# MyersGroup/relate

Measured on AMD Instinct MI355X. Metric: haplotype-pair*SNP updates/sec (Paint), higher is better.
Workload: dtype f64; 1 GPU; synthetic block-coalescent panel, N=5000 haplotypes x L=500000 SNPs, 1 chunk per GPU, 267 windows (--memory 20), Paint = PaintSteppingStones for all targets; sum_mode=exact, sum_k_D_k=264261546

## Files before the change

### include/relate_amd.h

```cpp
#ifndef RELATE_AMD_H
#define RELATE_AMD_H

#include <stddef.h>
#include <stdint.h>

#ifdef __cplusplus
extern "C" {
#endif

enum {
  RL_OK = 0,
  RL_EINVAL = -1,
  RL_ENODEVICE = -2,
  RL_EHIP = -3,
  RL_EIO = -4,
  RL_EFORMAT = -5,
  RL_ESTATE = -6,
  RL_ENOMEM = -7,
  RL_ETIMEOUT = -8
};

enum { RL_SUM_EXACT = 0, RL_SUM_LANES = 1, RL_SUM_EXACT_SERIAL = 2, RL_SUM_LANES32 = 3 };

typedef struct rl_ctx rl_ctx;
typedef struct rl_window rl_window;

const char *rl_last_error(void);
const char *rl_version(void);
int rl_device_count(void);

rl_ctx *rl_create(int device);
void rl_keep_cache_until_exit(int on);
void rl_destroy(rl_ctx *ctx);

int rl_load_chunk(rl_ctx *ctx, const char *dir, int chunk_index);

int rl_set_chunk(rl_ctx *ctx, int N, int L, const uint8_t *seq,
                 const double *r, const double *rpos, const int *wb, int W);
int rl_set_chunk_bits(rl_ctx *ctx, int N, int L, const uint32_t *bits,
                      int row_words, const double *r, const double *rpos,
                      const int *wb, int W);

int rl_set_painting(rl_ctx *ctx, double theta, double rho);

int rl_set_target_range(rl_ctx *ctx, int k_begin, int k_end);
int rl_target_range(const rl_ctx *ctx, int *k_begin, int *k_end);

int rl_set_window_range(rl_ctx *ctx, int w_first, int w_last);
int rl_window_range(const rl_ctx *ctx, int *w_first, int *w_last);

int rl_chunk_dims(const rl_ctx *ctx, int *N, int *L, int *W);
long long rl_total_sites(rl_ctx *ctx);

int rl_prepare(rl_ctx *ctx);

int rl_paint(rl_ctx *ctx, int sum_mode, float *kernel_ms);
int rl_set_paint_split(rl_ctx *ctx, int split);
int rl_set_paint_fit(rl_ctx *ctx, int fit);
int rl_set_paint_segments(rl_ctx *ctx, int backward, int forward);
int rl_paint_segments(rl_ctx *ctx, int *backward, int *forward);
int rl_paint_launched_segments(const rl_ctx *ctx, int *backward, int *forward);
int rl_paint_segment_range(int lo, int hi, int seg, int s, int *first, int *last);
int rl_tile_fit(int N, int *S, int *waves, int *tail, int *live);
int rl_paint_times(const rl_ctx *ctx, float *fwd_ms, float *bwd_ms);
int rl_paint_account(const rl_ctx *ctx, long long *fwd_steps, long long *bwd_steps, long long *stone_bytes);
int rl_register_tile(const rl_ctx *ctx, int *S, int *waves);

#define RL_DEBUG_SUM_STASH 0x100
#define RL_DEBUG_SUM_REGSTASH 0x200
int rl_debug_wave_sum(const double *x, int n, int batch, int sum_mode, double *out);
int rl_debug_wave_sum_ex(const double *x, int n, int batch, int rows_per_group, int sum_mode,
                         const uint8_t *mismatch, double th, double nth, double *out,
                         unsigned long long *stats8);
int rl_debug_term_split(int S, int *ks, int *r);
int rl_debug_walk_table(const int *A4, int p0, int sh, int delta_lo, int delta_hi, int *packable, int *out_table,
                        int *out_reference);

int rl_debug_stats(rl_ctx *ctx, unsigned long long *out16);
int rl_debug_stats32(rl_ctx *ctx, unsigned long long *out32);
int rl_debug_timeline(rl_ctx *ctx, unsigned long long *out, long long cap, long long *groups);

int rl_get_stones(rl_ctx *ctx, int w, float *alpha, float *beta,
                  float *ls_alpha, float *ls_beta, int *bsnp_begin,
                  int *bsnp_end);

int rl_write_paint_files(rl_ctx *ctx, const char *paint_dir);
int rl_write_paint_file(rl_ctx *ctx, int w, const char *path);
int rl_paint_record(rl_ctx *ctx, int w, int k, unsigned char *out, size_t cap, size_t *len);

int rl_stage_paint(const char *out_dir, int chunk_index, int use_painting,
                   double theta, double rho, int sum_mode, int device);

rl_window *rl_window_open(rl_ctx *ctx, int w, const char *paint_file,
                          int first_snp, int sum_mode, float *kernel_ms);
rl_window *rl_window_open_bounded(rl_ctx *ctx, int w, const char *paint_file,
                                  int first_snp, int sum_mode,
                                  long long max_rows, float *kernel_ms);
int rl_window_repaints(const rl_window *win);
void rl_window_close(rl_window *win);
int rl_window_bounds(const rl_window *win, int *start, int *end);
int rl_window_rows(const rl_window *win, int n);
int rl_window_get_topology(rl_window *win, int n, float *top,
                           float *logscales);

int rl_window_advance(rl_window *win, int snp);
int rl_window_matrix(rl_window *win, int snp, float *d_host, float *kernel_ms);
int rl_window_matrix_rows_device(rl_window *win, int snp, void *d_rows, float *kernel_ms);
int rl_window_matrix_rows_device_ex(rl_window *win, int snp, void *d_rows, const char *carriers, float val,
                                    void *d_rowmin, float *kernel_ms);

int rl_quickbuild(int N, double theta, float *d, const float *d_prior,
                  int *parent, int *child_left, int *child_right);
typedef struct rl_builder rl_builder;
rl_builder *rl_builder_create(int N, double theta, int device);
int rl_builder_build(rl_builder *b, float *d, const float *d_prior,
                     int *parent, int *child_left, int *child_right);
int rl_builder_set_sample_ages(rl_builder *b, const double *ages, int n);
int rl_builder_last_on_gpu(const rl_builder *b);
void rl_builder_destroy(rl_builder *b);
int rl_debug_rng_mismatches(unsigned seed, int n);
int rl_debug_builder_throughput(int N, double theta, int device, int builders, int reps, int workers, const float *d,
                                const float *prior, double *seconds, int *mismatches, int *first_parents);
int rl_debug_stage_worker_goal(int cus, int open_sections, int bounded_windows, int workers_per_cu);
int rl_debug_stage_plan(int N, int nloc, int S, int waves, const double *rows_of, int num_windows, int first_section,
                        int last_section, int stones_per_window, int gpu_build, int room_known, double room,
                        int host_threads, int window_rows_set, long long window_rows, long long window_parts,
                        int section_threads_set, long long section_threads, long long repaint_lanes, int probe_section,
                        long long *ints_out, double *doubles_out);

typedef struct rl_treeseq rl_treeseq;
typedef int (*rl_matrix_fn)(void *user, int snp, float *d);
typedef int (*rl_advance_fn)(void *user, int snp);
rl_treeseq *rl_treeseq_create(int N, int L, const uint32_t *bits, int row_words,
                              const double *rpos, const int *bp_pos,
                              const int *state, double theta);
void rl_treeseq_destroy(rl_treeseq *ts);
int rl_treeseq_set_sample_ages(rl_treeseq *ts, const double *ages, int n);
int rl_treeseq_set_build_device(rl_treeseq *ts, int device);
typedef int (*rl_matrix_dev_fn)(void *user, int snp, void *d_dev);
int rl_treeseq_set_device_matrix(rl_treeseq *ts, rl_matrix_dev_fn matrix_dev);
typedef int (*rl_matrix_dev_ex_fn)(void *user, int snp, void *d_matrix, const char *carriers, float val,
                                   void *d_rowmin);
int rl_treeseq_set_device_matrix_ex(rl_treeseq *ts, rl_matrix_dev_ex_fn matrix_dev_ex);
int rl_treeseq_build(rl_treeseq *ts, int start, int end, rl_matrix_fn matrix,
                     rl_advance_fn advance, void *user, int flags, int fb);
int rl_treeseq_num_trees(const rl_treeseq *ts);
int rl_treeseq_get_tree(const rl_treeseq *ts, int t, int *pos, int *parent);
int rl_treeseq_write(const rl_treeseq *ts, const char *anc_path,
                     const char *mut_path);

int rl_stage_build_topology(const char *out_dir, int chunk_index,
                            int first_section, int last_section,
                            int use_painting, double theta, double rho,
                            int flags, int fb, int sum_mode, int device);

typedef struct rl_stage_opts {
  size_t size;
  int sum_mode;
  int device;
// ... 123 lines not shown
```

### relate_amd/api.py

```python
import ctypes as C
import os

import numpy as np

_HERE = os.path.dirname(os.path.abspath(__file__))
LIB_PATH = os.path.join(_HERE, "librelate_amd.so")

RL_SUM_EXACT = 0
RL_SUM_LANES = 1
RL_SUM_EXACT_SERIAL = 2
RL_SUM_LANES32 = 3
RL_DEBUG_SUM_STASH = 0x100
RL_DEBUG_SUM_REGSTASH = 0x200

_lib = None


class RelateError(RuntimeError):
    pass


def lib():
    global _lib
    if _lib is None:
# ... 40 lines not shown
                                        C.c_void_p, C.POINTER(C.c_longlong)]
        L.rl_pairwise_anc.restype = C.c_int
        L.rl_pairwise_anc.argtypes = [C.POINTER(C.c_char_p), C.c_int, C.c_int, C.c_int, C.c_void_p,
                                      C.POINTER(C.c_longlong), C.POINTER(C.c_int)]
        L.rl_coalrate_batch_trees.argtypes = [C.c_int]
        L.rl_coalrate_epochs.argtypes = [C.c_float, C.c_char_p, C.c_void_p, C.POINTER(C.c_int)]
        L.rl_coalrate_trees.argtypes = [C.c_void_p, C.c_void_p, C.c_void_p, C.c_int, C.c_int, C.c_void_p, C.c_int,
                                        C.c_int, C.c_void_p]
        L.rl_coalrate_anc.argtypes = [C.c_char_p, C.c_char_p, C.c_void_p, C.c_int, C.c_int, C.c_void_p,
                                      C.POINTER(C.c_int)]
        L.rl_coalrate_write_bin.argtypes = [C.c_char_p, C.c_void_p, C.c_int, C.c_void_p, C.c_int]
        L.rl_coalrate_read_bin.argtypes = [C.c_char_p, C.c_void_p, C.POINTER(C.c_int), C.c_void_p, C.POINTER(C.c_int)]
        L.rl_coalrate_finalize.argtypes = [C.c_void_p, C.c_int, C.c_int, C.c_void_p, C.c_int, C.c_void_p]
        L.rl_coalrate_finalize_files.argtypes = [C.c_char_p, C.c_char_p, C.c_char_p]
        L.rl_window_copying.argtypes = [C.c_void_p, C.c_void_p, C.c_void_p]
        L.rl_window_copying_host.argtypes = [C.c_void_p, C.c_void_p, C.c_void_p]
        L.rl_copying_matrix.argtypes = [C.c_void_p, C.c_int, C.c_int, C.c_int, C.c_void_p, C.POINTER(C.c_longlong)]
        L.rl_copying_weights_host.argtypes = [C.c_void_p, C.c_int, C.c_void_p, C.c_int, C.c_int, C.c_void_p]
        L.rl_copying_rows_host.argtypes = [C.c_void_p, C.c_void_p, C.c_int, C.c_int, C.c_void_p]
        L.rl_stage_copying_matrix.argtypes = [C.c_char_p, C.c_int, C.c_int, C.c_int, C.c_void_p, C.c_char_p]
        _lib = L
    return _lib


class PaintTimeout(RelateError):
    """RL_ETIMEOUT: a segmented paint() gave up waiting for a hand-off"""


RL_ETIMEOUT = -8


def _check(rc):
    if rc == RL_ETIMEOUT:
        raise PaintTimeout("librelate_amd error %d: %s" % (rc, lib().rl_last_error().decode()))
    if rc != 0:
        raise RelateError("librelate_amd error %d: %s" % (rc, lib().rl_last_error().decode()))


def _p(a):
    return None if a is None else a.ctypes.data_as(C.c_void_p)


def device_count():
    return lib().rl_device_count()


def debug_wave_sum(x, sum_mode, rows_per_group=1, mismatch=None, th=0.001, nth=0.999, stash=False, regstash=False):
    if stash:
        sum_mode |= RL_DEBUG_SUM_STASH
    if regstash:
        sum_mode |= RL_DEBUG_SUM_REGSTASH
    x = np.ascontiguousarray(x, dtype=np.float64)
    batch, n = x.shape
    if mismatch is not None:
        mismatch = np.ascontiguousarray(mismatch, dtype=np.uint8)
        assert mismatch.shape == x.shape
    out = np.empty(batch, np.float64)
    st = np.zeros(8, np.uint64)
    f = lib().rl_debug_wave_sum_ex
    f.argtypes = [C.c_void_p, C.c_int, C.c_int, C.c_int, C.c_int, C.c_void_p, C.c_double, C.c_double, C.c_void_p,
                  C.c_void_p]
    _check(f(_p(x), n, batch, rows_per_group, sum_mode, _p(mismatch), th, nth, _p(out), _p(st)))
    return out, {"sums": int(st[0]), "fallbacks": int(st[1]), "walked": int(st[2]), "reruns": int(st[3])}


def term_split(S):
    ks, r = C.c_int(), C.c_int()
    _check(lib().rl_debug_term_split(int(S), C.byref(ks), C.byref(r)))
    return ks.value, r.value


def walk_table(A4, p0, sh, delta_lo, delta_hi):
    A4 = np.ascontiguousarray(A4, dtype=np.int32)
    assert A4.shape == (4,)
    n = int(delta_hi) - int(delta_lo) + 1
    tab, ref = np.empty(max(n, 0), np.int32), np.empty(max(n, 0), np.int32)
    ok = C.c_int()
    f = lib().rl_debug_walk_table
    f.argtypes = [C.c_void_p, C.c_int, C.c_int, C.c_int, C.c_int, C.POINTER(C.c_int), C.c_void_p, C.c_void_p]
    _check(f(_p(A4), int(p0), int(sh), int(delta_lo), int(delta_hi), C.byref(ok), _p(tab), _p(ref)))
    return bool(ok.value), tab, ref


def paint_segment_range(lo, hi, seg, s):
    a, b = C.c_int(), C.c_int()
    _check(lib().rl_paint_segment_range(int(lo), int(hi), int(seg), int(s), C.byref(a), C.byref(b)))
    return a.value, b.value


def tile_fit(N):
    s, w, t, l = C.c_int(), C.c_int(), C.c_int(), C.c_int()
    _check(lib().rl_tile_fit(int(N), C.byref(s), C.byref(w), C.byref(t), C.byref(l)))
    return s.value, w.value, t.value, l.value


class Context:

    def __init__(self, device=0):
        self._h = lib().rl_create(device)
        if not self._h:
            raise RelateError(lib().rl_last_error().decode())
        self.N = self.L = self.W = 0

    def close(self):
        if self._h:
            lib().rl_destroy(self._h)
            self._h = None

    def __del__(self):
        self.close()

    def _dims(self):
        n, l, w = C.c_int(), C.c_int(), C.c_int()
        _check(lib().rl_chunk_dims(C.c_void_p(self._h), C.byref(n), C.byref(l), C.byref(w)))
        self.N, self.L, self.W = n.value, l.value, w.value

    def load_chunk(self, out_dir, chunk_index=0):
        _check(lib().rl_load_chunk(C.c_void_p(self._h), out_dir.encode(), chunk_index))
        self._dims()

    def set_chunk(self, seq, r, rpos, wb):
        seq = np.ascontiguousarray(seq, dtype=np.uint8)
        L, N = seq.shape
        r = np.ascontiguousarray(r, dtype=np.float64)
        rpos = np.ascontiguousarray(rpos, dtype=np.float64)
        wb = np.ascontiguousarray(wb, dtype=np.int32)
        assert len(r) == L and len(rpos) == L + 1
        _check(lib().rl_set_chunk(C.c_void_p(self._h), N, L, _p(seq), _p(r), _p(rpos), _p(wb), len(wb) - 1))
        self._dims()

    def set_chunk_bits(self, N, bits, r, rpos, wb):
        bits = np.ascontiguousarray(bits, dtype=np.uint32)
        L, rw = bits.shape
        r = np.ascontiguousarray(r, dtype=np.float64)
        rpos = np.ascontiguousarray(rpos, dtype=np.float64)
        wb = np.ascontiguousarray(wb, dtype=np.int32)
        _check(lib().rl_set_chunk_bits(C.c_void_p(self._h), N, L, _p(bits), rw, _p(r), _p(rpos), _p(wb),
                                       len(wb) - 1))
        self._dims()

    def set_painting(self, theta, rho):
        _check(lib().rl_set_painting(C.c_void_p(self._h), theta, rho))

    def set_target_range(self, k_begin, k_end):
        _check(lib().rl_set_target_range(C.c_void_p(self._h), int(k_begin), int(k_end)))

    def target_range(self):
        a, b = C.c_int(), C.c_int()
        _check(lib().rl_target_range(C.c_void_p(self._h), C.byref(a), C.byref(b)))
        return a.value, b.value

    def set_window_range(self, w_first, w_last):
        _check(lib().rl_set_window_range(C.c_void_p(self._h), int(w_first), int(w_last)))

    def window_range(self):
        a, b = C.c_int(), C.c_int()
        _check(lib().rl_window_range(C.c_void_p(self._h), C.byref(a), C.byref(b)))
        return a.value, b.value

    def paint_account(self):
        f, b, n = C.c_longlong(0), C.c_longlong(0), C.c_longlong(0)
        _check(lib().rl_paint_account(C.c_void_p(self._h), C.byref(f), C.byref(b), C.byref(n)))
        return f.value, b.value, n.value

    def total_sites(self):
        v = lib().rl_total_sites(C.c_void_p(self._h))
# ... 603 lines not shown
```

### relate_amd/csrc/debug_kernels.hip

```cpp
#define RL_STATS 1
#include "paint_device.h"
#include "exact_sum.h"
#include "launch.h"
#include "common.h"

#include <vector>

namespace rl {

constexpr int SUM_STATS = 8;

enum { TERM_REG = 0, TERM_MASK = 1, TERM_STASH = 2, TERM_REGSTASH = 3 };

template <int S, int MODE, int WAVES, int KIND>
__global__ void __launch_bounds__(64 * WAVES) sum_kernel(const double *__restrict__ x, int n, int rows_per_group,
                                                         const unsigned long long *__restrict__ masks, double th,
                                                         double nth, double *__restrict__ out,
                                                         unsigned long long *__restrict__ stats) {
  __shared__ WaveLinkStorage link;
  __shared__ unsigned long long lstats[SUM_STATS];
  constexpr bool STASHING = KIND == TERM_STASH || KIND == TERM_REGSTASH;
  constexpr int STASH = STASHING ? stash_bytes(S) : 16;
  constexpr int R = KIND == TERM_REGSTASH ? reg_stash_terms(S) : 0;
  __shared__ __attribute__((aligned(16))) char stash[WAVES][STASH];
// ... 106 lines not shown
  const Layout lay = make_layout(n, waves);
  const int S = choose_S(lay);
  if (!S) {
    set_error("rl_debug_wave_sum_ex: no register tile for n=%d", n);
    return RL_EINVAL;
  }
  std::vector<unsigned long long> masks;
  if (mismatch) {
    masks.assign((size_t)batch * waves * S, 0ull);
    for (size_t b = 0; b < (size_t)batch; b++)
      for (int vl = 0; vl < 64 * waves; vl++) {
        const int start = vl * lay.q + (vl < lay.rem ? vl : lay.rem), len = lay.q + (vl < lay.rem ? 1 : 0);
        unsigned long long *words = &masks[(b * waves + vl / 64) * S];
        for (int j = 0; j < len; j++)
          if (mismatch[b * n + start + j]) words[j] |= 1ull << (vl & 63);
      }
  }
  DevBuf dx, dout, dmask, dstats;
  int rc;
  if ((rc = dx.alloc(sizeof(double) * (size_t)n * batch))) return rc;
  if ((rc = dout.alloc(sizeof(double) * batch))) return rc;
  if ((rc = dstats.alloc(sizeof(unsigned long long) * SUM_STATS))) return rc;
  if (mismatch && (rc = dmask.alloc(sizeof(unsigned long long) * masks.size()))) return rc;
  RL_HIP(hipMemcpy(dx.p, x, sizeof(double) * (size_t)n * batch, hipMemcpyHostToDevice));
  RL_HIP(hipMemset(dstats.p, 0, sizeof(unsigned long long) * SUM_STATS));
  if (mismatch)
    RL_HIP(hipMemcpy(dmask.p, masks.data(), sizeof(unsigned long long) * masks.size(), hipMemcpyHostToDevice));
  const unsigned long long *dm = mismatch ? dmask.as<unsigned long long>() : nullptr;
  const int groups = batch / rows_per_group;
  hipError_t e;
  switch (kernel_mode(sum_mode)) {
#define RL_ARGS S, waves, dx.as<double>(), n, groups, rows_per_group, dm, th, nth, dout.as<double>(), \
                dstats.as<unsigned long long>(), kind
    case 0: e = launch_sum<0>(RL_ARGS); break;
    case 1: e = launch_sum<1>(RL_ARGS); break;
    default: e = launch_sum<2>(RL_ARGS); break;
#undef RL_ARGS
  }
  RL_HIP(e);
  RL_HIP(hipDeviceSynchronize());
  RL_HIP(hipMemcpy(out, dout.p, sizeof(double) * batch, hipMemcpyDeviceToHost));
  if (stats8) RL_HIP(hipMemcpy(stats8, dstats.p, sizeof(unsigned long long) * SUM_STATS, hipMemcpyDeviceToHost));
  return RL_OK;
}

extern "C" int rl_debug_wave_sum(const double *x, int n, int batch, int sum_mode, double *out) {
  return rl_debug_wave_sum_ex(x, n, batch, 1, sum_mode, nullptr, 0.0, 0.0, out, nullptr);
}

extern "C" int rl_debug_term_split(int S, int *ks, int *r) {
  using namespace rl;
  const hipError_t e = dispatch_tile(S, 1, [&](auto s, auto, auto) {
    *ks = stash_terms(s());
    *r = reg_stash_terms(s());
    return hipSuccess;
  });
  if (e != hipSuccess) {
    set_error("rl_debug_term_split: no register tile S=%d", S);
    return RL_EINVAL;
  }
  return RL_OK;
}

extern "C" int rl_debug_walk_table(const int *A4, int p0, int sh, int delta_lo, int delta_hi, int *packable,
                                   int *out_table, int *out_reference) {
  using namespace rl;
  if (!A4 || !packable || !out_table || !out_reference) {
    set_error("rl_debug_walk_table: null argument");
    return RL_EINVAL;
  }
  if (p0 < 0 || p0 > 3 || sh < 0 || sh > 1 || delta_hi < delta_lo) {
    set_error("rl_debug_walk_table: p0=%d outside 0..3, sh=%d outside 0..1 or delta_hi=%d < delta_lo=%d", p0, sh,
              delta_hi, delta_lo);
    return RL_EINVAL;
  }
  const WalkTable t = walk_table_pack(A4[0], A4[1], A4[2], A4[3], p0, sh);
  *packable = t.ok ? 1 : 0;
  for (long long d = delta_lo; d <= delta_hi; d++) {
    out_reference[d - delta_lo] = walk_hop_reference(A4[0], A4[1], A4[2], A4[3], p0, sh, (int)d);
    out_table[d - delta_lo] = t.ok ? walk_table_hop(t.lo, t.hi, 16 * p0, sh, (int)d) : 0;
  }
  return RL_OK;
}
```

### relate_amd/csrc/exact_sum.h

```cpp
#pragma once
#include "paint_device.h"

namespace rl {

template <int CTRL, int ROW_MASK = 0xf, int BANK_MASK = 0xf>
RL_DEV double dpp_f64(double v) {
  const long long b = __double_as_longlong(v);
  const int lo = __builtin_amdgcn_update_dpp(0, (int)b, CTRL, ROW_MASK, BANK_MASK, true);
  const int hi = __builtin_amdgcn_update_dpp(0, (int)(b >> 32), CTRL, ROW_MASK, BANK_MASK, true);
  return __longlong_as_double(((long long)hi << 32) | (unsigned int)lo);
}
template <int CTRL, int ROW_MASK = 0xf, int BANK_MASK = 0xf>
RL_DEV int dpp_i32(int v) {
  return __builtin_amdgcn_update_dpp(0, v, CTRL, ROW_MASK, BANK_MASK, true);
}
enum { DPP_ROW_SHR = 0x110, DPP_WAVE_SHR1 = 0x138, DPP_ROW_BCAST15 = 0x142, DPP_ROW_BCAST31 = 0x143 };

RL_DEV double wave_scan_f64(double v) {
  v += dpp_f64<DPP_ROW_SHR + 1>(v);
  v += dpp_f64<DPP_ROW_SHR + 2>(v);
  v += dpp_f64<DPP_ROW_SHR + 4>(v);
  v += dpp_f64<DPP_ROW_SHR + 8>(v);
  v += dpp_f64<DPP_ROW_BCAST15, 0xa>(v);
  v += dpp_f64<DPP_ROW_BCAST31, 0xc>(v);
  return v;
}
RL_DEV int hi32(double v) { return (int)(__double_as_longlong(v) >> 32); }
RL_DEV int expo_field(double v) { return (hi32(v) >> 20) & 0x7ff; }
RL_DEV double rd_lane_f64(double v, int lane) {
  const long long b = __double_as_longlong(v);
  const int lo = __builtin_amdgcn_readlane((int)b, lane);
  const int hi = __builtin_amdgcn_readlane((int)(b >> 32), lane);
  return __longlong_as_double(((long long)hi << 32) | (unsigned int)lo);
}
RL_DEV double pow2_field(int f) { return __longlong_as_double((long long)f << 52); }

template <int S, int LIVE = S>
struct RegTerm {
  static constexpr bool REG = true;
  const double (&a)[S];
  double th = 0.0, nth = 0.0;
  unsigned long long *stats = nullptr;
  RL_DEV double get(int i, double, double) const { return a[i]; }
  template <typename F>
  RL_DEV void for_each(double &, double &, F &&f) const {
#pragma unroll
    for (int i = 0; i < LIVE; i++) f(i, a[i]);
  }
};
template <int S, int LIVE = S>
struct MaskTerm {
  static constexpr bool REG = false;
  MaskRow row;
  const double (&b)[S];
  double th, nth;
  unsigned long long *stats = nullptr;
  template <typename F>
  RL_DEV void for_each(double &t, double &n, F &&f) const {
    for_each_chunk<S, 4>(row, [&](int j0, const u64x4 &m) {
      double x[4];
      if (j0 + 4 <= LIVE)
        weighted4(x, b[j0], b[j0 + 1], b[j0 + 2], b[j0 + 3], m, t, n);
      else
        weighted3(x, b[j0], b[j0 + 1], b[j0 + 2], m, t, n);
#pragma unroll
      for (int jj = 0; jj < 4; jj++)
        if (j0 + jj < LIVE) f(j0 + jj, x[jj]);
    });
  }
};

constexpr int STASH_MAX = 36;
constexpr int LDS_PER_CU = 160 * 1024;
constexpr int stash_terms(int S) {
  const int fit = (LDS_PER_CU / (4 * tile_waves_per_simd(S)) - 512) / (64 * (int)sizeof(double));
  const int ks = fit < S ? fit : S;
  return (ks < STASH_MAX ? ks : STASH_MAX) / 4 * 4;
}
constexpr int stash_bytes(int S) { return stash_terms(S) * 64 * (int)sizeof(double); }
constexpr int reg_stash_terms(int S) { return S == 80 ? 12 : S == 64 ? 28 : 0; }
template <int S, int R>
RL_DEV void hold_term(double (&xr)[R > 0 ? R : 1], int i, double x) {
  if constexpr (R > 0)
    if (i >= S - R) xr[i - (S - R)] = x;
}
constexpr int STASH_AHEAD = 2;
typedef double f64x2 __attribute__((ext_vector_type(2)));
typedef f64x2 __attribute__((may_alias)) StashPair;
typedef __attribute__((address_space(3))) StashPair *StashPtr;
RL_DEV StashPtr stash_of(void *wave_region) { return (StashPtr)wave_region + (threadIdx.x & 63); }
RL_DEV void stash_put4(StashPtr sp, int chunk, const double (&x)[4]) {
  StashPair lo, hi;
  lo.x = x[0]; lo.y = x[1]; hi.x = x[2]; hi.y = x[3];
  sp[128 * chunk] = lo;
  sp[128 * chunk + 64] = hi;
}
RL_DEV void stash_put3(StashPtr sp, int chunk, const double (&x)[4]) {
  StashPair lo;
  lo.x = x[0]; lo.y = x[1];
  sp[128 * chunk] = lo;
  *(__attribute__((address_space(3))) double __attribute__((may_alias)) *)&sp[128 * chunk + 64] = x[2];
}
template <int S, int LIVE = S, int R = reg_stash_terms(S)>
struct StashTerm {
  static constexpr bool REG = false;
  static constexpr int KS = stash_terms(S);
  static_assert(R % 4 == 0 && KS + R <= S, "the register-held chunks lie behind the stashed ones");
// ... 70 lines not shown
  lk.w = WAVES > 1 ? __builtin_amdgcn_readfirstlane((int)(threadIdx.x >> 6)) : 0;
  return lk;
}
template <int WAVES>
RL_DEV double lanes_total(double lane_sum, WaveLink<WAVES> &lk) {
  lk.phase++;
  const double t = wave_sum_butterfly(lane_sum);
  if constexpr (WAVES == 1) {
    return t;
  } else {
    const unsigned ph = lk.phase & 1u;
    if ((threadIdx.x & 63) == 0) lk.s->tot[ph][lk.w] = t;
    lk.barrier();
    return lk.s->tot[ph][0] + lk.s->tot[ph][1];
  }
}

template <int S, typename T>
RL_DEV double sum_exact_fallback(const T &term, double s = 0.0) {
  for (int l = 0; l < 64; l++) {
    double th = term.th, nth = term.nth;
    double tmp = s;
    term.for_each(th, nth, [&](int, double x) {
      tmp += x;
      if constexpr (!T::REG) asm volatile("" : "+v"(th), "+v"(nth), "+v"(tmp));
    });
    s = wave_bcast(tmp, l);
  }
  return s;
}
template <int S, int WAVES, typename T>
RL_DEV double sum_exact_fallback_linked(const T &term, const WaveLink<WAVES> &lk) {
  if constexpr (WAVES == 1) {
    return sum_exact_fallback<S>(term);
  } else {
    double r = 0.0;
    if (lk.w == 0) {
      r = sum_exact_fallback<S>(term);
      if ((threadIdx.x & 63) == 0) lk.s->result = r;
    }
    lk.barrier();
    if (lk.w == 1) {
      r = sum_exact_fallback<S>(term, lk.s->result);
    }
    lk.barrier();
    if (lk.w == 1 && (threadIdx.x & 63) == 0) lk.s->result = r;
    lk.barrier();
    r = lk.s->result;
    lk.barrier();
    return r;
  }
}

constexpr int WALK_G4 = 16384;
RL_HD inline int walk_hop_reference(int A0, int A1, int A2, int A3, int p0, int sh, int delta) {
  const int h = (p0 + delta) & 3;
  const int A = (h & 2) ? ((h & 1) ? A3 : A2) : ((h & 1) ? A1 : A0);
  const int B = h == 0 ? (-p0 - WALK_G4) : (h == 3 ? (3 - p0 + WALK_G4) : (h - p0));
  return A + ((delta - B) >> sh);
}
RL_HD inline int walk_run_offset(int A, int h, int p0, int sh) {
  const int B = h - p0 + (h == 0 ? -WALK_G4 : h == 3 ? WALK_G4 : 0);
  return A - (B >> sh);
}
struct WalkTable {
  int lo, hi;
  bool ok;
};
RL_HD inline WalkTable walk_table_pack_runs(int U0, int U1, int U2, int U3) {
  WalkTable t;
  t.ok = (short)U0 == U0 && (short)U1 == U1 && (short)U2 == U2 && (short)U3 == U3;
  t.lo = (int)(((unsigned)U0 & 0xffffu) | ((unsigned)U1 << 16));
  t.hi = (int)(((unsigned)U2 & 0xffffu) | ((unsigned)U3 << 16));
  return t;
}
RL_HD inline WalkTable walk_table_pack(int A0, int A1, int A2, int A3, int p0, int sh) {
  return walk_table_pack_runs(walk_run_offset(A0, 0, p0, sh), walk_run_offset(A1, 1, p0, sh),
                              walk_run_offset(A2, 2, p0, sh), walk_run_offset(A3, 3, p0, sh));
}
RL_HD inline int walk_table_hop(int lo, int hi, int p16, int sh, int delta) {
  const unsigned long long t = ((unsigned long long)(unsigned)hi << 32) | (unsigned)lo;
  return (delta >> sh) + (int)(short)(unsigned short)(t >> (((delta << 4) + p16) & 48));
}

#ifdef RL_STATS
#define RL_CLK() __builtin_readcyclecounter()
#define RL_STAT(i, v) do { if (term.stats && (threadIdx.x & 63) == 0) atomicAdd(&term.stats[i], (unsigned long long)(v)); } while (0)
#else
#define RL_CLK() 0ull
#define RL_STAT(i, v) do { } while (0)
#endif

template <int S, int WAVES, typename T>
RL_DEV double sum_exact_fast(const T &term, double L, WaveLink<WAVES> &lk) {
  constexpr bool REG_TERM = T::REG;
  constexpr int G4 = WALK_G4;

  const unsigned long long tk0 = RL_CLK();
  double Q = wave_scan_f64(L);
  double P = dpp_f64<DPP_WAVE_SHR1>(Q);
  if constexpr (WAVES > 1) {
    const int lane = threadIdx.x & 63;
    const unsigned ph = lk.phase & 1u;
    if (lane == 63) lk.s->tot[ph][lk.w] = Q;
    lk.barrier();
    if (lk.w == 1) {
      const double before = lk.s->tot[ph][0];
      Q = before + Q;
      P = dpp_f64<DPP_WAVE_SHR1>(Q);
      if (lane == 0) P = before;
    }
  }
  const long long pb = __double_as_longlong(P);
  const bool zero_entry = pb == 0 || ((threadIdx.x & 63) == 1 && lk.w == 0);

  const unsigned long long tk1 = RL_CLK();
  const long long base = pb & ~3ll;
  const int p0 = (int)(pb & 3);
  double c0 = __longlong_as_double(base - G4);
  double c1 = __longlong_as_double(base + 1);
  double c2 = __longlong_as_double(base + 2);
  double c3 = __longlong_as_double(base + 3 + G4);
  if (zero_entry) { c0 = P; c1 = P; c2 = P; c3 = P; }
  const double r0 = c0, r3 = c3;
  const int e_in = expo_field(r0);
  const bool entry_ok = zero_entry || (e_in == expo_field(r3) && e_in > 64);
  int exdiff = 0;
  double thB = term.th, nthB = term.nth;
  term.for_each(thB, nthB, [&](int, double x) {
    c0 += x;
    c1 += x;
    c2 += x;
    c3 += x;
    exdiff = __builtin_amdgcn_bitop3_b32(exdiff, hi32(c0), hi32(c3), 0xF6);
    if constexpr (REG_TERM)
      __builtin_amdgcn_sched_barrier(0);
    else
      asm volatile("" : "+v"(exdiff), "+v"(c1), "+v"(c2), "+v"(thB), "+v"(nthB));
  });
  const unsigned long long tk2 = RL_CLK();
  const int e_out = expo_field(c0);
  const int e_next = expo_field(Q);
  const unsigned q_lo = (unsigned)__double_as_longlong(Q);
  auto exit_offset = [&](double c) -> int { return (int)((unsigned)__double_as_longlong(c) - q_lo); };

  const bool same_seq = (exdiff >> 20) == 0;
  const int sh = e_out - e_in;
  bool invalid = !entry_ok || !same_seq;
  if (!zero_entry && e_out != e_next) invalid = true;
  if (zero_entry && expo_field(c0) != e_next) invalid = true;
  const bool jump = !zero_entry && !invalid && sh >= 2;
  const bool constant = jump && __double_as_longlong(c0) == __double_as_longlong(c3);
  const bool special = jump && !constant;

  int A0 = 0;
  if (constant) A0 = exit_offset(c0);
  if (zero_entry && __double_as_longlong(c0) != __double_as_longlong(Q)) A0 = exit_offset(c0);
  int mK = 0, mC = zero_entry ? A0 : 0;
  bool affine = zero_entry;
  const bool table = !invalid && !jump && !zero_entry;
  int U0 = A0, U1 = 0, U2 = 0, U3 = 0;
  if (table) {
    U0 = walk_run_offset(exit_offset(c0), 0, p0, sh);
    U1 = walk_run_offset(exit_offset(c1), 1, p0, sh);
    U2 = walk_run_offset(exit_offset(c2), 2, p0, sh);
    U3 = walk_run_offset(exit_offset(c3), 3, p0, sh);
    const int e = p0 & 1;
    const bool k0 = U0 == U1 && U1 == U2 && U2 == U3;
    const bool k1 = sh != 0 && U0 == U2 && U1 == U3 && U0 - U1 == 2 * e - 1;
    affine = k0 || k1;
    mK = k0 ? 0 : 1;
    mC = k0 ? U0 : U0 - e;
  }
  const int mS = (affine && !zero_entry) ? sh : 0;
  if (!affine) { mK = 0; mC = 0; }
  const WalkTable wt = walk_table_pack_runs(U0, U1, U2, U3);
  const bool redo = special || !wt.ok;
  const int t01 = wt.lo, t23 = wt.hi;
  const int meta = (p0 << 4) | (sh << 2) | (redo ? 1 : 0);

  const double Qt = rd_lane_f64(Q, 63);
  {
    const long long qb = __double_as_longlong(Qt) & ~3ll;
    const int ea = expo_field(__longlong_as_double(qb - G4)), eb = expo_field(__longlong_as_double(qb + 3 + G4));
    if (ea != eb || ea <= 64) invalid = true;
  }
  int sK = mK, sC = mC, sS = affine ? mS : (64 | (meta << 8));
  auto combine = [&](int pK, int pC, int pS) {
    if (!(sS & 64)) {
      const int ps = pS & 63;
      sK = pK + ((pC + sK) << ps);
      sS = (ps + (sS & 63)) | (pS & 64);
    }
  };
#define RL_SCAN_STEP(CTRL, RM)                                              \
  {                                                                         \
    const int pK = __builtin_amdgcn_update_dpp(0, sK, CTRL, RM, 0xf, true); \
    const int pC = __builtin_amdgcn_update_dpp(0, sC, CTRL, RM, 0xf, true); \
    const int pS = __builtin_amdgcn_update_dpp(0, sS, CTRL, RM, 0xf, true); \
    combine(pK, pC, pS);                                                    \
  }
  RL_SCAN_STEP(DPP_ROW_SHR + 1, 0xf)
  RL_SCAN_STEP(DPP_ROW_SHR + 2, 0xf)
  RL_SCAN_STEP(DPP_ROW_SHR + 4, 0xf)
  RL_SCAN_STEP(DPP_ROW_SHR + 8, 0xf)
  RL_SCAN_STEP(DPP_ROW_BCAST15, 0xa)
  RL_SCAN_STEP(DPP_ROW_BCAST31, 0xc)
#undef RL_SCAN_STEP
  RL_STAT(0, 1);
  bool fallback = __ballot(invalid || (sS & 63) > 20) != 0ull;
  if constexpr (WAVES > 1) {
    if ((threadIdx.x & 63) == 0) lk.s->bad[lk.w] = fallback;
    lk.barrier();
    fallback = lk.s->bad[0] | lk.s->bad[1];
  }
  if (fallback) {
    RL_STAT(1, 1);
    return sum_exact_fallback_linked<S, WAVES>(term, lk);
  }
  const unsigned long long tk3 = RL_CLK();
  unsigned long long todo = __ballot(!affine);
  RL_STAT(2, __builtin_popcountll(todo));
  {
    const unsigned long long sp = __ballot(special || (table && !affine && !wt.ok));
    (void)sp;
    RL_STAT(3, __builtin_popcountll(sp));
  }
  int delta = 0;
  if constexpr (WAVES > 1) {
    if (lk.w == 1) {
      lk.barrier();
      delta = lk.s->delta;
    }
  }
  {
    const unsigned long long cm = __ballot(constant);
    if (cm) {
      const int qc = 63 - __builtin_clzll(cm);
      delta = (int)(short)__builtin_amdgcn_readlane(t01, qc);
      todo &= ~((2ull << qc) - 1ull);
    }
  }
  while (todo) {
    const int q = __builtin_ctzll(todo);
    todo &= todo - 1;
    const int tlo = __builtin_amdgcn_readlane(t01, q), thi = __builtin_amdgcn_readlane(t23, q);
    const int m = __builtin_amdgcn_readlane(sS, q) >> 8;
    if (WAVES == 1 || q > 0) {
      const int K = __builtin_amdgcn_readlane(sK, q - 1), C = __builtin_amdgcn_readlane(sC, q - 1);
      const int sft = __builtin_amdgcn_readlane(sS, q - 1) & 63;
      delta = ((delta + K) >> sft) + C;
    }
    if (m & 1) {
      const double Pq = rd_lane_f64(P, q);
      const double uq = pow2_field(expo_field(Pq) - 52);
      double t = Pq + (double)delta * uq;
      double thC = term.th, nthC = term.nth;
      term.for_each(thC, nthC, [&](int, double x) {
        t += x;
        if constexpr (!REG_TERM) asm volatile("" : "+v"(thC), "+v"(nthC));
      });
      const double v = rd_lane_f64(t, q);
      delta = (int)((unsigned)__double_as_longlong(v) - (unsigned)__builtin_amdgcn_readlane((int)q_lo, q));
    } else {
      delta = walk_table_hop(tlo, thi, m & 48, (m >> 2) & 1, delta);
    }
  }
  {
    const int K = __builtin_amdgcn_readlane(sK, 63), C = __builtin_amdgcn_readlane(sC, 63);
    const int sft = __builtin_amdgcn_readlane(sS, 63) & 63;
    delta = ((delta + K) >> sft) + C;
  }
  {
    const unsigned long long tk4 = RL_CLK();
    (void)tk0; (void)tk1; (void)tk2; (void)tk3; (void)tk4;
    RL_STAT(4, tk1 - tk0);
    RL_STAT(5, tk2 - tk1);
    RL_STAT(6, tk3 - tk2);
    RL_STAT(7, tk4 - tk3);
  }
  if constexpr (WAVES > 1) {
    const int lane = threadIdx.x & 63;
    if (lk.w == 0) {
      if (lane == 0) lk.s->delta = delta;
      lk.barrier();
      lk.barrier();
    } else {
      if (lane == 0) lk.s->result = Qt + (double)delta * pow2_field(expo_field(Qt) - 52);
      lk.barrier();
    }
    const double r = lk.s->result;
    lk.barrier();
    return r;
  }
  return Qt + (double)delta * pow2_field(expo_field(Qt) - 52);
}

template <int MODE, int S, int WAVES, typename T>
RL_DEV double wave_sum(const T &term, double L, WaveLink<WAVES> &lk) {
  if constexpr (MODE == 0) {
    return lanes_total(L, lk);
  } else {
    lk.phase++;
    if constexpr (MODE == 1)
      return sum_exact_fast<S, WAVES>(term, L, lk);
    else
      return sum_exact_fallback_linked<S, WAVES>(term, lk);
  }
}
template <int MODE, int S, typename T>
RL_DEV double wave_sum(const T &term, double L) {
  WaveLink<1> lk;
  return wave_sum<MODE, S, 1>(term, L, lk);
}

template <int S, typename T>
RL_DEV double local_sum(const T &term) {
  double L = 0.0, th = term.th, nth = term.nth;
  term.for_each(th, nth, [&](int, double x) { L += x; });
  return L;
}

}
```

Baseline: 2191 billion updates/s.

## Replace affine segmented walk with translation-scan plus serial table hops in single-wave exact sum

For single-wave exact summation, the carry walk now folds pure-translation lanes into an integer wave prefix scan (DPP u32 scan). It then walks only the non-translation lanes serially via readlane, using packed int16 hop tables, and recomputes per-lane terms only for special lanes. The older affine-composition path is kept for multi-wave blocks. The aim is to cut the per-wave carry resolution work, at the cost of a serial loop whose length depends on how many lanes are not translations. A host debug reference is added to check the new walk.

New measurement: 2264 billion updates/s, median of 6. +3.3%, better.

```diff
diff --git a/include/relate_amd.h b/include/relate_amd.h
--- a/include/relate_amd.h
+++ b/include/relate_amd.h
@@ -75,6 +75,10 @@
 int rl_debug_term_split(int S, int *ks, int *r);
 int rl_debug_walk_table(const int *A4, int p0, int sh, int delta_lo, int delta_hi, int *packable, int *out_table,
                         int *out_reference);
+#define RL_WALK_TRANSLATION 0
+#define RL_WALK_TABLE 1
+#define RL_WALK_CONSTANT 2
+int rl_debug_walk_lanes(const int *records, int lanes, int entry_delta, int *out_literal, int *out_scan);
 
 int rl_debug_stats(rl_ctx *ctx, unsigned long long *out16);
 int rl_debug_stats32(rl_ctx *ctx, unsigned long long *out32);
diff --git a/relate_amd/api.py b/relate_amd/api.py
--- a/relate_amd/api.py
+++ b/relate_amd/api.py
@@ -146,6 +146,19 @@
     return bool(ok.value), tab, ref
 
 
+WALK_TRANSLATION, WALK_TABLE, WALK_CONSTANT = 0, 1, 2
+
+
+def walk_lanes(records, entry_delta=0):
+    records = np.ascontiguousarray(records, dtype=np.int32)
+    assert records.ndim == 2 and records.shape[1] == 7
+    lit, scan = C.c_int(), C.c_int()
+    f = lib().rl_debug_walk_lanes
+    f.argtypes = [C.c_void_p, C.c_int, C.c_int, C.POINTER(C.c_int), C.POINTER(C.c_int)]
+    _check(f(_p(records), int(records.shape[0]), int(entry_delta), C.byref(lit), C.byref(scan)))
+    return lit.value, scan.value
+
+
 def paint_segment_range(lo, hi, seg, s):
     a, b = C.c_int(), C.c_int()
     _check(lib().rl_paint_segment_range(int(lo), int(hi), int(seg), int(s), C.byref(a), C.byref(b)))
diff --git a/relate_amd/csrc/debug_kernels.hip b/relate_amd/csrc/debug_kernels.hip
--- a/relate_amd/csrc/debug_kernels.hip
+++ b/relate_amd/csrc/debug_kernels.hip
@@ -212,3 +212,75 @@
   }
   return RL_OK;
 }
+
+extern "C" int rl_debug_walk_lanes(const int *records, int lanes, int entry_delta, int *out_literal, int *out_scan) {
+  using namespace rl;
+  if (!records || !out_literal || !out_scan) {
+    set_error("rl_debug_walk_lanes: null argument");
+    return RL_EINVAL;
+  }
+  if (lanes < 1 || lanes > 64) {
+    set_error("rl_debug_walk_lanes: lanes=%d outside 1..64", lanes);
+    return RL_EINVAL;
+  }
+  for (int l = 0; l < lanes; l++) {
+    const int *r = records + 7 * l;
+    if (r[0] < RL_WALK_TRANSLATION || r[0] > RL_WALK_CONSTANT) {
+      set_error("rl_debug_walk_lanes: lane %d: kind=%d outside 0..2", l, r[0]);
+      return RL_EINVAL;
+    }
+    if (r[0] == RL_WALK_TABLE &&
+        (r[5] < 0 || r[5] > 3 || r[6] < 0 || r[6] > 1 || !walk_table_pack_runs(r[1], r[2], r[3], r[4]).ok)) {
+      set_error("rl_debug_walk_lanes: lane %d: p0=%d outside 0..3, sh=%d outside 0..1 or a U_h that is no int16", l,
+                r[5], r[6]);
+      return RL_EINVAL;
+    }
+    if (r[0] == RL_WALK_CONSTANT && (short)r[1] != r[1]) {
+      set_error("rl_debug_walk_lanes: lane %d: the exit offset %d of a constant lane is no int16", l, r[1]);
+      return RL_EINVAL;
+    }
+  }
+  int delta = entry_delta;
+  for (int l = 0; l < lanes; l++) {
+    const int *r = records + 7 * l;
+    if (r[0] == RL_WALK_TRANSLATION) {
+      delta = (int)((unsigned)delta + (unsigned)r[1]);
+    } else if (r[0] == RL_WALK_CONSTANT) {
+      delta = r[1];
+    } else {
+      int A[4];
+      for (int h = 0; h < 4; h++) A[h] = r[1 + h] - walk_run_offset(0, h, r[5], r[6]);
+      delta = walk_hop_reference(A[0], A[1], A[2], A[3], r[5], r[6], delta);
+    }
+  }
+  *out_literal = delta;
+  unsigned T[64], run = 0;
+  unsigned long long todo = 0;
+  int qc = -1;
+  for (int l = 0; l < lanes; l++) {
+    const int *r = records + 7 * l;
+    if (r[0] == RL_WALK_TRANSLATION)
+      run += (unsigned)r[1];
+    else
+      todo |= 1ull << l;
+    if (r[0] == RL_WALK_CONSTANT) qc = l;
+    T[l] = run;
+  }
+  int rel = entry_delta;
+  if (qc >= 0) {
+    rel = walk_leave((int)(short)walk_table_pack_runs(records[7 * qc + 1], 0, 0, 0).lo, T[qc]);
+    todo &= ~((2ull << qc) - 1ull);
+  }
+  while (todo) {
+    const int q = __builtin_ctzll(todo);
+    todo &= todo - 1;
+    const int *r = records + 7 * q;
+    const WalkTable t = walk_table_pack_runs(r[1], r[2], r[3], r[4]);
+    const int m = walk_meta(r[5], r[6], false);
+    delta = walk_enter(rel, T[q]);
+    delta = walk_head_hop(t.lo, t.hi, m, delta);
+    rel = walk_leave(delta, T[q]);
+  }
+  *out_scan = walk_enter(rel, T[lanes - 1]);
+  return RL_OK;
+}
diff --git a/relate_amd/csrc/exact_sum.h b/relate_amd/csrc/exact_sum.h
--- a/relate_amd/csrc/exact_sum.h
+++ b/relate_amd/csrc/exact_sum.h
@@ -23,6 +23,15 @@
   v += dpp_f64<DPP_ROW_SHR + 8>(v);
   v += dpp_f64<DPP_ROW_BCAST15, 0xa>(v);
   v += dpp_f64<DPP_ROW_BCAST31, 0xc>(v);
+  return v;
+}
+RL_DEV unsigned wave_scan_u32(unsigned v) {
+  v += (unsigned)dpp_i32<DPP_ROW_SHR + 1>((int)v);
+  v += (unsigned)dpp_i32<DPP_ROW_SHR + 2>((int)v);
+  v += (unsigned)dpp_i32<DPP_ROW_SHR + 4>((int)v);
+  v += (unsigned)dpp_i32<DPP_ROW_SHR + 8>((int)v);
+  v += (unsigned)dpp_i32<DPP_ROW_BCAST15, 0xa>((int)v);
+  v += (unsigned)dpp_i32<DPP_ROW_BCAST31, 0xc>((int)v);
   return v;
 }
 RL_DEV int hi32(double v) { return (int)(__double_as_longlong(v) >> 32); }
@@ -259,6 +268,17 @@
   const unsigned long long t = ((unsigned long long)(unsigned)hi << 32) | (unsigned)lo;
   return (delta >> sh) + (int)(short)(unsigned short)(t >> (((delta << 4) + p16) & 48));
 }
+enum { WALK_META_REDO = 64, WALK_META_SH_BIT = 7 };
+RL_HD inline int walk_meta(int p0, int sh, bool redo) {
+  return (p0 << 4) | (redo ? WALK_META_REDO : 0) | (sh << WALK_META_SH_BIT);
+}
+RL_HD inline int walk_head_hop(int lo, int hi, int meta, int delta) {
+  const unsigned long long t = ((unsigned long long)(unsigned)hi << 32) | (unsigned)lo;
+  return (delta >> ((meta >> WALK_META_SH_BIT) & 1)) + (int)(short)(unsigned short)(t >> (((delta << 4) + meta) & 63));
+}
+
+RL_HD inline int walk_enter(int rel, unsigned T) { return (int)((unsigned)rel + T); }
+RL_HD inline int walk_leave(int delta, unsigned T) { return (int)((unsigned)delta - T); }
 
 #ifdef RL_STATS
 #define RL_CLK() __builtin_readcyclecounter()
@@ -268,28 +288,16 @@
 #define RL_STAT(i, v) do { } while (0)
 #endif
 
-template <int S, int WAVES, typename T>
-RL_DEV double sum_exact_fast(const T &term, double L, WaveLink<WAVES> &lk) {
+template <int S, typename T>
+RL_DEV double sum_exact_fast(const T &term, double L) {
   constexpr bool REG_TERM = T::REG;
   constexpr int G4 = WALK_G4;
 
   const unsigned long long tk0 = RL_CLK();
   double Q = wave_scan_f64(L);
   double P = dpp_f64<DPP_WAVE_SHR1>(Q);
-  if constexpr (WAVES > 1) {
-    const int lane = threadIdx.x & 63;
-    const unsigned ph = lk.phase & 1u;
-    if (lane == 63) lk.s->tot[ph][lk.w] = Q;
-    lk.barrier();
-    if (lk.w == 1) {
-      const double before = lk.s->tot[ph][0];
-      Q = before + Q;
-      P = dpp_f64<DPP_WAVE_SHR1>(Q);
-      if (lane == 0) P = before;
-    }
-  }
   const long long pb = __double_as_longlong(P);
-  const bool zero_entry = pb == 0 || ((threadIdx.x & 63) == 1 && lk.w == 0);
+  const bool zero_entry = pb == 0 || (threadIdx.x & 63) == 1;
 
   const unsigned long long tk1 = RL_CLK();
   const long long base = pb & ~3ll;
@@ -333,6 +341,150 @@
   int A0 = 0;
   if (constant) A0 = exit_offset(c0);
   if (zero_entry && __double_as_longlong(c0) != __double_as_longlong(Q)) A0 = exit_offset(c0);
+  const bool table = !invalid && !jump && !zero_entry;
+  int U0 = A0, U1 = 0, U2 = 0, U3 = 0;
+  bool translation = zero_entry;
+  if (table) {
+    U0 = walk_run_offset(exit_offset(c0), 0, p0, sh);
+    U1 = walk_run_offset(exit_offset(c1), 1, p0, sh);
+    U2 = walk_run_offset(exit_offset(c2), 2, p0, sh);
+    U3 = walk_run_offset(exit_offset(c3), 3, p0, sh);
+    translation = sh == 0 && U0 == U1 && U1 == U2 && U2 == U3;
+  }
+  const WalkTable wt = walk_table_pack_runs(U0, U1, U2, U3);
+  const bool redo = special || !wt.ok;
+  const int t01 = wt.lo, t23 = wt.hi;
+  const int meta = walk_meta(p0, sh, redo);
+
+  const double Qt = rd_lane_f64(Q, 63);
+  {
+    const long long qb = __double_as_longlong(Qt) & ~3ll;
+    const int ea = expo_field(__longlong_as_double(qb - G4)), eb = expo_field(__longlong_as_double(qb + 3 + G4));
+    if (ea != eb || ea <= 64) invalid = true;
+  }
+  const unsigned TS = wave_scan_u32(translation ? (unsigned)U0 : 0u);
+  RL_STAT(0, 1);
+  if (__ballot(invalid) != 0ull) {
+    RL_STAT(1, 1);
+    return sum_exact_fallback<S>(term);
+  }
+  const unsigned long long tk3 = RL_CLK();
+  unsigned long long todo = __ballot(!translation);
+  RL_STAT(2, __builtin_popcountll(todo));
+  {
+    const unsigned long long sp = __ballot(special || (table && !translation && !wt.ok));
+    (void)sp;
+    RL_STAT(3, __builtin_popcountll(sp));
+  }
+  int rel = 0;
+  {
+    const unsigned long long cm = __ballot(constant);
+    if (cm) {
+      const int qc = 63 - __builtin_clzll(cm);
+      rel = walk_leave((int)(short)__builtin_amdgcn_readlane(t01, qc),
+                       (unsigned)__builtin_amdgcn_readlane((int)TS, qc));
+      todo &= ~((2ull << qc) - 1ull);
+    }
+  }
+  while (todo) {
+    const int q = __builtin_ctzll(todo);
+    asm("s_bitset0_b64 %0, %1" : "+s"(todo) : "s"(q));
+    const int tlo = __builtin_amdgcn_readlane(t01, q), thi = __builtin_amdgcn_readlane(t23, q);
+    const int m = __builtin_amdgcn_readlane(meta, q);
+    const unsigned Tq = (unsigned)__builtin_amdgcn_readlane((int)TS, q);
+    const int din = walk_enter(rel, Tq);
+    int dout = walk_head_hop(tlo, thi, m, din);
+    if (m & WALK_META_REDO) {
+      const double Pq = rd_lane_f64(P, q);
+      const double uq = pow2_field(expo_field(Pq) - 52);
+      double t = Pq + (double)din * uq;
+      double thC = term.th, nthC = term.nth;
+      term.for_each(thC, nthC, [&](int, double x) {
+        t += x;
+        if constexpr (!REG_TERM) asm volatile("" : "+v"(thC), "+v"(nthC));
+      });
+      const double v = rd_lane_f64(t, q);
+      dout = (int)((unsigned)__double_as_longlong(v) - (unsigned)__builtin_amdgcn_readlane((int)q_lo, q));
+    }
+    rel = walk_leave(dout, Tq);
+  }
+  const int delta = walk_enter(rel, (unsigned)__builtin_amdgcn_readlane((int)TS, 63));
+  {
+    const unsigned long long tk4 = RL_CLK();
+    (void)tk0; (void)tk1; (void)tk2; (void)tk3; (void)tk4;
+    RL_STAT(4, tk1 - tk0);
+    RL_STAT(5, tk2 - tk1);
+    RL_STAT(6, tk3 - tk2);
+    RL_STAT(7, tk4 - tk3);
+  }
+  return Qt + (double)delta * pow2_field(expo_field(Qt) - 52);
+}
+
+template <int S, int WAVES, typename T>
+RL_DEV double sum_exact_fast_segmented(const T &term, double L, WaveLink<WAVES> &lk) {
+  constexpr bool REG_TERM = T::REG;
+  constexpr int G4 = WALK_G4;
+
+  const unsigned long long tk0 = RL_CLK();
+  double Q = wave_scan_f64(L);
+  double P = dpp_f64<DPP_WAVE_SHR1>(Q);
+  if constexpr (WAVES > 1) {
+    const int lane = threadIdx.x & 63;
+    const unsigned ph = lk.phase & 1u;
+    if (lane == 63) lk.s->tot[ph][lk.w] = Q;
+    lk.barrier();
+    if (lk.w == 1) {
+      const double before = lk.s->tot[ph][0];
+      Q = before + Q;
+      P = dpp_f64<DPP_WAVE_SHR1>(Q);
+      if (lane == 0) P = before;
+    }
+  }
+  const long long pb = __double_as_longlong(P);
+  const bool zero_entry = pb == 0 || ((threadIdx.x & 63) == 1 && lk.w == 0);
+
+  const unsigned long long tk1 = RL_CLK();
+  const long long base = pb & ~3ll;
+  const int p0 = (int)(pb & 3);
+  double c0 = __longlong_as_double(base - G4);
+  double c1 = __longlong_as_double(base + 1);
+  double c2 = __longlong_as_double(base + 2);
+  double c3 = __longlong_as_double(base + 3 + G4);
+  if (zero_entry) { c0 = P; c1 = P; c2 = P; c3 = P; }
+  const double r0 = c0, r3 = c3;
+  const int e_in = expo_field(r0);
+  const bool entry_ok = zero_entry || (e_in == expo_field(r3) && e_in > 64);
+  int exdiff = 0;
+  double thB = term.th, nthB = term.nth;
+  term.for_each(thB, nthB, [&](int, double x) {
+    c0 += x;
+    c1 += x;
+    c2 += x;
+    c3 += x;
+    exdiff = __builtin_amdgcn_bitop3_b32(exdiff, hi32(c0), hi32(c3), 0xF6);
+    if constexpr (REG_TERM)
+      __builtin_amdgcn_sched_barrier(0);
+    else
+      asm volatile("" : "+v"(exdiff), "+v"(c1), "+v"(c2), "+v"(thB), "+v"(nthB));
+  });
+  const unsigned long long tk2 = RL_CLK();
+  const int e_out = expo_field(c0);
+  const int e_next = expo_field(Q);
+  const unsigned q_lo = (unsigned)__double_as_longlong(Q);
+  auto exit_offset = [&](double c) -> int { return (int)((unsigned)__double_as_longlong(c) - q_lo); };
+
+  const bool same_seq = (exdiff >> 20) == 0;
+  const int sh = e_out - e_in;
+  bool invalid = !entry_ok || !same_seq;
+  if (!zero_entry && e_out != e_next) invalid = true;
+  if (zero_entry && expo_field(c0) != e_next) invalid = true;
+  const bool jump = !zero_entry && !invalid && sh >= 2;
+  const bool constant = jump && __double_as_longlong(c0) == __double_as_longlong(c3);
+  const bool special = jump && !constant;
+
+  int A0 = 0;
+  if (constant) A0 = exit_offset(c0);
+  if (zero_entry && __double_as_longlong(c0) != __double_as_longlong(Q)) A0 = exit_offset(c0);
   int mK = 0, mC = zero_entry ? A0 : 0;
   bool affine = zero_entry;
   const bool table = !invalid && !jump && !zero_entry;
@@ -479,8 +631,10 @@
     return lanes_total(L, lk);
   } else {
     lk.phase++;
-    if constexpr (MODE == 1)
-      return sum_exact_fast<S, WAVES>(term, L, lk);
+    if constexpr (MODE == 1 && WAVES == 1)
+      return sum_exact_fast<S>(term, L);
+    else if constexpr (MODE == 1)
+      return sum_exact_fast_segmented<S, WAVES>(term, L, lk);
     else
       return sum_exact_fallback_linked<S, WAVES>(term, lk);
   }
```
